# luisdiaz1997/GPzoo

Measured on AMD Instinct MI355X. Metric: ELBO evals/sec (L=32-latent evaluations, all GPUs) at M=2048 inducing, N=200000, L=32 latents/GPU x 1 GPU(s), higher is better.
Workload: dtype f32; 1 GPU; BASELINE configs[2]: Slide-seq-shaped synthetic, N=200000 spots, M=2048, L=32 latents/GPU x 1 GPU(s), matern32, f32; latents_total=32, whitened=True, chunk=0, factor_dtype=f64

## Files before the change

### gpzoo_amd/csrc/gemmw.hip

```cpp
#include "gemmw.h"

#include "cov.h"


#include <cmath>
#include <mutex>
#include <type_traits>
#include <utility>

#ifndef GPZ_W_ABL
#define GPZ_W_ABL 0
#endif

namespace gpz {

typedef float f32x4 __attribute__((ext_vector_type(4)));

enum { WB_MEM = 0, WB_GEN = 1 };
enum { WA_DENSE = 0, WA_LOWER = 1, WA_UPPER = 2 };
enum { WE_STORE_STATS = 0,
       WE_STATS = 1,
       WE_STORE = 2,
       WE_STORE_COLSCALE = 3,
       WE_WBAR = 4,
       WE_KBAR = 5,
       WE_ADD_COLSCALE = 6 };

struct WParams {
  const float* A; int64_t lda, sA0;
  const float* B; int64_t ldb, sB0;
  const float* Z; int64_t MD;
  const float* X; int64_t nreal;
  const float* sigma; const float* ell;
  float* C; int64_t ldc, sC0;
  const float* mu; int64_t sMu;
  float* ps_sq; float* ps_mu; int64_t ncols;
  const float* colscale; const float* colvec; int64_t sCs;
  const float* rowvec; int64_t sRv;
  const float* aux;
  int64_t M;
  int L, nblk, mtw, nt, W, strips;
  int pair, colmajor;
  const int32_t* gate;
};

constexpr int W_BK = 16;

template <int TM, int TN, int BSRC, int D>
struct WLds {
  static constexpr int A_ELEMS = TM * W_BK;
  static constexpr int RPP = 256 / TN;
  static constexpr int PITCH = 256 + (RPP == 2 ? 8 : RPP == 1 ? 4 : 16);
  static constexpr int B_ELEMS = (W_BK / RPP) * PITCH;
  static constexpr int STAGE = A_ELEMS + B_ELEMS;
  static constexpr int ZB = 128 * D;
  static constexpr size_t bytes = sizeof(float) * (2 * STAGE + (BSRC == WB_GEN ? 2 * ZB : 0));
};

template <int TM, int TN, int BSRC, int ATRI, int EPI, int KIND, int D>
__global__ __launch_bounds__(64 * (TM / 128) * (TN / 32)) __attribute__((amdgpu_waves_per_eu(4, 4))) void gemmw_kernel(const WParams p) {
  constexpr int BK = W_BK;
  if (p.gate && *p.gate == 0) return;
  constexpr int WMW = TM / 128, WNW = TN / 32;
  constexpr int NW = WMW * WNW;
  static_assert(NW == 8 || NW == 16, "8 or 16 waves of 128 x 32");
  using G = WLds<TM, TN, BSRC, D>;
  constexpr int RPP = G::RPP, PITCH = G::PITCH;
  extern __shared__ __attribute__((aligned(1024))) char smem_raw[];
  float* const smem = reinterpret_cast<float*>(smem_raw);
  auto sA = [&](int buf) -> float* { return smem + buf * G::STAGE; };
  auto sB = [&](int buf) -> float* { return smem + buf * G::STAGE + G::A_ELEMS; };
  float* const sZ = smem + 2 * G::STAGE;
  auto addrB = [](int k, int n) { return (k / RPP) * PITCH + (k % RPP) * TN + n; };

  int tj, b0, leg_ti[2], nlegs = 1;
  {
    const int bid = blockIdx.x;
    const int x = bid & 7, s = bid >> 3;
    if (BSRC == WB_GEN) {
      const int ug = s / p.W, within = s - ug * p.W;
      const int u = ug * 8 + x;
      const int per_level = p.L * p.strips;
      if (u >= p.mtw * per_level) return;
      const int level = u / per_level, rem = u - level * per_level;
      leg_ti[0] = leg_ti[1] = (ATRI == WA_LOWER) ? p.mtw - 1 - level : level;
      b0 = rem / p.strips;
      tj = (rem - b0 * p.strips) * p.W + within;
    } else {
      const int per_unit = (p.pair ? (p.mtw + 1) >> 1 : p.mtw) * p.W;
      const int u = (s / per_unit) * 8 + x, within = s % per_unit;
      if (u >= p.L * p.strips) return;
      b0 = u / p.strips;
      const int nrow = p.pair ? (p.mtw + 1) >> 1 : p.mtw;
      const int pi = p.colmajor ? within % nrow : within / p.W, far = p.pair ? p.mtw - 1 - pi : pi;
      const int strip = u - b0 * p.strips, c0 = strip * p.nt / p.strips, c1 = (strip + 1) * p.nt / p.strips;
      tj = c0 + (p.colmajor ? within / nrow : within % p.W);
      if (tj >= c1) return;
      const bool long_first = ((s >> 5) & 1) == 0;
      leg_ti[0] = ((ATRI == WA_LOWER) == long_first) ? far : pi;
      leg_ti[1] = ((ATRI == WA_LOWER) == long_first) ? pi : far;
      nlegs = far == pi ? 1 : 2;
      if (!p.pair) leg_ti[0] = leg_ti[1] = (ATRI == WA_LOWER) ? p.mtw - 1 - pi : pi;
    }
    if (tj >= p.nt) return;
  }
  const int tid = threadIdx.x, lane = tid & 63;
  const int wave = __builtin_amdgcn_readfirstlane(tid >> 6);
  const int wn = wave % WNW;
  const int r = lane & 15, q = lane >> 4;
  const int Mp = p.nblk * 128;

  typedef __attribute__((address_space(3))) void lds_void;
  constexpr int NPA = TM / (16 * NW);
#if defined(__HIP_DEVICE_COMPILE__)
  const __amdgpu_buffer_rsrc_t a_rsrc = __builtin_amdgcn_make_buffer_rsrc(
      const_cast<float*>(p.A + b0 * p.sA0), 0, (int)(p.lda * Mp * sizeof(float)), 0x00020000);
  const __amdgpu_buffer_rsrc_t b_rsrc = __builtin_amdgcn_make_buffer_rsrc(
      const_cast<float*>(BSRC == WB_MEM ? p.B + b0 * p.sB0 : p.Z), 0,
      (int)((BSRC == WB_MEM ? p.ldb * Mp : p.MD) * sizeof(float)), 0x00020000);
#endif
  auto k_begin_of = [&](int ti) { return (ATRI == WA_UPPER) ? TM * ti : 0; };
  auto k_end_of = [&](int ti) { return (ATRI == WA_LOWER) ? min(TM * (ti + 1), Mp) : Mp; };
  int a_soff[NPA], b_soff = 0;
  auto gperm = [](int w) { const int t = (w >> 2) & 3; return (((t >> 1) ^ t) & 1) << 1 | (t >> 1); };
  const int a_voff = ((lane >> 2) * (int)p.lda + (((lane & 3) ^ gperm(lane >> 2)) * 4)) * (int)sizeof(float);
  const int b_voff = ((lane / (TN / 4)) * (int)p.ldb + (lane % (TN / 4)) * 4) * (int)sizeof(float);
  bool abl_first = true;
  auto stage_load = [&](int buf) __attribute__((always_inline)) {
    if ((GPZ_W_ABL & 2) && !abl_first) return;
    abl_first = false;
#if defined(__HIP_DEVICE_COMPILE__)
#pragma unroll
    for (int h = 0; h < NPA; ++h) {
      __builtin_amdgcn_raw_ptr_buffer_load_lds(a_rsrc, (lds_void*)(sA(buf) + (NPA * wave + h) * 256), 16, a_voff, a_soff[h], 0, 0);
      a_soff[h] += BK * (int)sizeof(float);
    }
    if constexpr (BSRC == WB_MEM) {
      constexpr int NPB = (W_BK / RPP) / NW;
      static_assert(BSRC != WB_MEM || (NPB * NW * RPP == W_BK && NPB >= 1), "whole B pieces per wave");
#pragma unroll
      for (int h = 0; h < NPB; ++h)
        __builtin_amdgcn_raw_ptr_buffer_load_lds(b_rsrc, (lds_void*)(sB(buf) + (wave + NW * h) * PITCH), 16, b_voff,
                                                 b_soff + h * NW * RPP * (int)p.ldb * (int)sizeof(float), 0, 0);
      b_soff += BK * (int)p.ldb * (int)sizeof(float);
    }
#endif
  };
  auto tile_begin = [&](int ti) __attribute__((always_inline)) {
    const int kb = k_begin_of(ti);
#pragma unroll
    for (int h = 0; h < NPA; ++h) {
      int row = ti * TM + (NPA * wave + h) * 16;
      while (row >= Mp) row -= 128;
      a_soff[h] = (row * (int)p.lda + kb) * (int)sizeof(float);
    }
    b_soff = ((kb + RPP * wave) * (int)p.ldb + tj * TN) * (int)sizeof(float);
    stage_load(0);
  };

  constexpr int NXC = TN / 64;
  float xc[NXC][D], ampn[NXC], c0n[NXC];
  CovConst cc = {0.f, 0.f, 0.f};
  if constexpr (BSRC == WB_GEN) {
    cc = cov_const<KIND>(p.sigma[b0], p.ell[b0]);
#pragma unroll
    for (int h = 0; h < NXC; ++h) {
      const int64_t n = (int64_t)tj * TN + h * 64 + lane;
      const bool real = n < p.nreal;
#pragma unroll
      for (int k = 0; k < D; ++k) xc[h][k] = real ? p.X[n * D + k] : 0.f;
      ampn[h] = real ? cc.amp : 0.f;
      c0n[h] = (KIND == 1 && !real) ? 0.f : cc.c0;
    }
  }
  auto z_load = [&](int blk) __attribute__((always_inline)) {
#if defined(__HIP_DEVICE_COMPILE__)
    if (wave < 2 * D)
      __builtin_amdgcn_raw_ptr_buffer_load_lds(b_rsrc, (lds_void*)(sZ + (blk & 1) * G::ZB + wave * 64), 4, lane * 4,
                                               (blk * G::ZB + wave * 64) * 4, 0, 0);
#endif
  };
  auto b_generate = [&](int buf, int step) __attribute__((always_inline)) {
#pragma unroll
    for (int i = 0; i < BK / NW; ++i) {
      const int kk = wave + NW * i, kg = step * BK + kk;
      const float* zp = sZ + ((kg >> 7) & 1) * G::ZB + (kg & 127) * D;
      float z[D];
#pragma unroll
      for (int k = 0; k < D; ++k) z[k] = zp[k];
#pragma unroll
      for (int h = 0; h < NXC; ++h) {
        const float v = (GPZ_W_ABL & 1) ? z[0] + xc[h][0]
                                        : cov_value<KIND>(cov_radial<KIND>(cov_d2<D>(z, xc[h])), ampn[h], c0n[h], cc.c1);
        sB(buf)[addrB(kk, h * 64 + lane)] = v;
      }
    }
  };

  f32x4 acc[8][2];

  int wm = 0, nk = 0, db = 0, n_a = 0, fr_a = 0, step0 = 0, t = 0, next_ti = -1;
  bool active = false;
  int fr_b[4];
#pragma unroll
  for (int j = 0; j < 4; ++j) fr_b[j] = addrB(4 * q + j, wn * 32 + r);

  auto mma_step = [&](int buf, auto lo_c, auto hi_c) __attribute__((always_inline)) {
    constexpr int LO = decltype(lo_c)::value, HI = decltype(hi_c)::value;
    float bf[4][2];
#pragma unroll
    for (int j = 0; j < 4; ++j)
#pragma unroll
      for (int ni = 0; ni < 2; ++ni) bf[j][ni] = sB(buf)[fr_b[j] + ni * 16];
#pragma unroll
    for (int half = 0; half < 2; ++half) {
      f32x4 fa[4];
#pragma unroll
      for (int m = 0; m < 4; ++m)
        if (half * 4 + m >= LO && half * 4 + m <= HI)
          fa[m] = *reinterpret_cast<const f32x4*>(sA(buf) + fr_a + (half * 4 + m) * 16 * BK);
#pragma unroll
      for (int j = 0; j < 4; ++j)
#pragma unroll
        for (int m = 0; m < 4; ++m)
#pragma unroll
          for (int ni = 0; ni < 2; ++ni)
            if (half * 4 + m >= LO && half * 4 + m <= HI)
              acc[half * 4 + m][ni] = __builtin_amdgcn_mfma_f32_16x16x4f32(fa[m][j], bf[j][ni], acc[half * 4 + m][ni], 0, 0, 0);
    }
  };

  using std::integral_constant;
  auto step = [&](auto par_c, auto run_c, auto lo_c, auto hi_c) __attribute__((always_inline)) {
    constexpr int P = decltype(par_c)::value;
    if (t + 1 < nk) {
      stage_load(P ^ 1);
      if constexpr (BSRC == WB_GEN) {
        const int st = step0 + t;
        if ((st & 7) == 0 && (st >> 3) + 1 < p.nblk) z_load((st >> 3) + 1);
        b_generate(P ^ 1, st + 1);
      }
    } else if (next_ti >= 0) {
      tile_begin(next_ti);
    }
    if constexpr (decltype(run_c)::value) mma_step(P, lo_c, hi_c);
    if (GPZ_W_ABL & 16) {
      asm volatile("s_waitcnt lgkmcnt(0)" ::: "memory");
      __builtin_amdgcn_s_barrier();
    } else {
      asm volatile("s_waitcnt vmcnt(0)" ::: "memory");
      if (!(GPZ_W_ABL & 8)) __syncthreads();
    }
    ++t;
  };
  using no_run = integral_constant<bool, false>;
  using run = integral_constant<bool, true>;
  using i0 = integral_constant<int, 0>;
  using i1 = integral_constant<int, 1>;
  using i7 = integral_constant<int, 7>;
  auto idle_until = [&](int end) __attribute__((always_inline)) {
    while (t < end) { step(i0{}, no_run{}, i0{}, i7{}); step(i1{}, no_run{}, i0{}, i7{}); }
  };
  auto full_until = [&](int end) __attribute__((always_inline)) {
    while (t < end) { step(i0{}, run{}, i0{}, i7{}); step(i1{}, run{}, i0{}, i7{}); }
  };
  auto diagonal = [&](auto self, auto u_c) __attribute__((always_inline)) -> void {
    constexpr int U = decltype(u_c)::value;
    if constexpr (ATRI == WA_LOWER) step(integral_constant<int, U & 1>{}, run{}, integral_constant<int, U>{}, i7{});
    else step(integral_constant<int, U & 1>{}, run{}, i0{}, integral_constant<int, U>{});
    if constexpr (U + 1 < 8) self(self, integral_constant<int, U + 1>{});
  };

  tile_begin(leg_ti[0]);
#pragma unroll 1
  for (int leg = 0; leg < nlegs; ++leg) {
    const int ti = leg_ti[leg];
    wm = WMW == 1 ? 0 : (wave / WNW) ^ ((ti ^ tj) & 1);
    const int k_begin = k_begin_of(ti);
    nk = (k_end_of(ti) - k_begin) / BK;
    db = WMW * ti + wm;
    active = db < p.nblk && (int64_t)tj * TN + wn * 32 < p.ncols;
    n_a = 8 * (ATRI == WA_LOWER ? db : wm);
    fr_a = (wm * 128 + r) * BK + ((q ^ gperm(r)) * 4);
    step0 = k_begin / BK;
    t = 0;
    next_ti = leg + 1 < nlegs ? leg_ti[leg + 1] : -1;
#pragma unroll
    for (int mi = 0; mi < 8; ++mi)
#pragma unroll
      for (int ni = 0; ni < 2; ++ni) acc[mi][ni] = f32x4{0, 0, 0, 0};
    if constexpr (BSRC == WB_GEN) {
      z_load(step0 >> 3);
      asm volatile("s_waitcnt vmcnt(0)" ::: "memory");
      __syncthreads();
      b_generate(0, step0);
    }
    if (leg == 0) asm volatile("s_waitcnt vmcnt(0)" ::: "memory");
    asm volatile("s_waitcnt lgkmcnt(0)" ::: "memory");
    __builtin_amdgcn_s_barrier();
    if (!active) {
      idle_until(nk);
    } else if constexpr (ATRI == WA_DENSE) {
      full_until(nk);
    } else if constexpr (ATRI == WA_LOWER) {
      full_until(n_a);
      diagonal(diagonal, i0{});
      idle_until(nk);
    } else {
      idle_until(n_a);
      diagonal(diagonal, i0{});
      full_until(nk);
    }

    if (!active) continue;
    if (GPZ_W_ABL & 4) {
      float sum = 0.f;
#pragma unroll
      for (int mi = 0; mi < 8; ++mi)
#pragma unroll
        for (int ni = 0; ni < 2; ++ni)
#pragma unroll
          for (int g = 0; g < 4; ++g) sum += acc[mi][ni][g];
      if (sum == 12345.678f) p.ps_sq[0] = sum;
      continue;
    }
    const int64_t row0 = (int64_t)db * 128;
    const int64_t ccol0 = (int64_t)tj * TN + wn * 32;
    if (BSRC == WB_GEN && row0 + 128 > p.M) {
#pragma unroll
      for (int mi = 0; mi < 8; ++mi)
#pragma unroll
        for (int g = 0; g < 4; ++g)
          if (row0 + mi * 16 + 4 * q + g >= p.M) {
#pragma unroll
            for (int ni = 0; ni < 2; ++ni) acc[mi][ni][g] = 0.f;
          }
    }
    if constexpr (EPI == WE_STORE_STATS || EPI == WE_STATS) {
      float ssq[2] = {0.f, 0.f}, smu[2] = {0.f, 0.f};
#pragma unroll
      for (int mi = 0; mi < 8; ++mi) {
        f32x4 m4 = {0, 0, 0, 0};
        if constexpr (EPI == WE_STORE_STATS) m4 = *reinterpret_cast<const f32x4*>(p.mu + b0 * p.sMu + row0 + 4 * q + mi * 16);
#pragma unroll
        for (int g = 0; g < 4; ++g)
#pragma unroll
          for (int ni = 0; ni < 2; ++ni) {
            const float v = acc[mi][ni][g];
            ssq[ni] = __builtin_fmaf(v, v, ssq[ni]);
            if constexpr (EPI == WE_STORE_STATS) smu[ni] = __builtin_fmaf(m4[g], v, smu[ni]);
          }
      }
#pragma unroll
      for (int ni = 0; ni < 2; ++ni) {
        ssq[ni] += __shfl_xor(ssq[ni], 16); ssq[ni] += __shfl_xor(ssq[ni], 32);
        if constexpr (EPI == WE_STORE_STATS) { smu[ni] += __shfl_xor(smu[ni], 16); smu[ni] += __shfl_xor(smu[ni], 32); }
        if (q == 0) {
          const int64_t o = ((int64_t)b0 * p.nblk + db) * p.ncols + ccol0 + ni * 16 + r;
          p.ps_sq[o] = ssq[ni];
          if constexpr (EPI == WE_STORE_STATS) p.ps_mu[o] = smu[ni];
        }
      }
    }
    if constexpr (EPI != WE_STATS) {
      constexpr int LDE = 36;
      static_assert(NW * 16 * LDE <= G::STAGE, "the epilogue strips fit tile buffer 1");
      float* strip = sA(1) + wave * (16 * LDE);
      float* Cg = p.C + b0 * p.sC0 + row0 * p.ldc + ccol0;
      int srow = lane >> 3;
      asm volatile("" : "+v"(srow));
      const int c4 = (lane & 7) * 4;
      float cs[2] = {1.f, 1.f};
      if constexpr (EPI == WE_STORE_COLSCALE) {
#pragma unroll
        for (int ni = 0; ni < 2; ++ni) cs[ni] = p.colscale[b0 * p.sCs + ccol0 + ni * 16 + r];
      }
      f32x4 sc = {0, 0, 0, 0}, cv = {0, 0, 0, 0};
      if constexpr (EPI == WE_WBAR || EPI == WE_KBAR || EPI == WE_ADD_COLSCALE)
        sc = *reinterpret_cast<const f32x4*>(p.colscale + b0 * p.sCs + ccol0 + c4);
      if constexpr (EPI == WE_WBAR || EPI == WE_KBAR)
        cv = *reinterpret_cast<const f32x4*>(p.colvec + b0 * p.sCs + ccol0 + c4);
#pragma unroll
      for (int mi = 0; mi < 8; ++mi) {
#pragma unroll
        for (int ni = 0; ni < 2; ++ni)
#pragma unroll
          for (int g = 0; g < 4; ++g) strip[(4 * q + g) * LDE + ni * 16 + r] = cs[ni] * acc[mi][ni][g];
        __builtin_amdgcn_wave_barrier();
        f32x4 w[2];
        float rv[2];
        if constexpr (EPI == WE_WBAR || EPI == WE_KBAR || EPI == WE_ADD_COLSCALE) {
#pragma unroll
          for (int it = 0; it < 2; ++it) {
            const int64_t row = mi * 16 + it * 8 + srow;
            if constexpr (EPI == WE_WBAR) w[it] = *reinterpret_cast<const f32x4*>(p.aux + b0 * p.sC0 + (row0 + row) * p.ldc + ccol0 + c4);
            if constexpr (EPI == WE_ADD_COLSCALE) w[it] = *reinterpret_cast<const f32x4*>(Cg + (int64_t)row * p.ldc + c4);
            if constexpr (EPI != WE_ADD_COLSCALE) rv[it] = p.rowvec[b0 * p.sRv + row0 + row];
          }
        }
#pragma unroll
        for (int it = 0; it < 2; ++it) {
          const int row = it * 8 + srow;
          f32x4 v = *reinterpret_cast<const f32x4*>(strip + row * LDE + c4);
          if constexpr (EPI == WE_WBAR) {
#pragma unroll
            for (int e = 0; e < 4; ++e) v[e] = v[e] + rv[it] * cv[e] - w[it][e] * sc[e];
          }
          if constexpr (EPI == WE_KBAR) {
#pragma unroll
            for (int e = 0; e < 4; ++e) v[e] = v[e] * sc[e] + rv[it] * cv[e];
          }
          if constexpr (EPI == WE_ADD_COLSCALE) {
#pragma unroll
            for (int e = 0; e < 4; ++e) v[e] = w[it][e] + v[e] * sc[e];
          }
          *reinterpret_cast<f32x4*>(Cg + (int64_t)(mi * 16 + row) * p.ldc + c4) = v;
        }
        __builtin_amdgcn_wave_barrier();
      }
    }
  }
}

struct NTParams {
  const float* A; const float* B; float* C;
  int64_t ld, sAB, ldc, sC;
  int K, nblk, mt, L, T;
  int S, Ks;
  float* part; int64_t sPart;
  const float* w; int64_t sW;
  const int32_t* gate;
  const float* gm; float* vpart;
};

template <int TM, bool WTS>
__global__ __launch_bounds__(TM * 2) __attribute__((amdgpu_waves_per_eu(4, 4))) void gemmw_nt_kernel(const NTParams p) {
  constexpr int BK = W_BK, TN = 128;
  if (p.gate && *p.gate == 0) return;
  constexpr int NW = TM / 32;
  constexpr int A_ELEMS = TM * BK, B_ELEMS = TN * BK, STAGE = A_ELEMS + B_ELEMS;
  extern __shared__ __attribute__((aligned(1024))) char smem_raw[];
  float* const smem = reinterpret_cast<float*>(smem_raw);
  auto sA = [&](int buf) -> float* { return smem + buf * STAGE; };
  auto sB = [&](int buf) -> float* { return smem + buf * STAGE + A_ELEMS; };
  int b0, ti, tj, piece;
  {
    const int nb = (int)gridDim.x, qn = nb >> 3, rem = nb & 7, x = blockIdx.x & 7;
    const int lid0 = x * qn + min(x, rem) + (int)(blockIdx.x >> 3);
    const int grp = lid0 / p.T;
    const int t = lid0 - grp * p.T;
    b0 = grp / p.S;
    piece = grp - b0 * p.S;
    if constexpr (TM == 256) {
      int i = (int)((sqrtf(4.0f * (float)t + 1.0f) - 1.0f) * 0.5f);
      while ((i + 1) * (i + 2) <= t) ++i;
      while (i * (i + 1) > t) --i;
      ti = i; tj = t - i * (i + 1);
    } else {
      int i = (int)((sqrtf(8.0f * (float)t + 1.0f) - 1.0f) * 0.5f);
      while ((i + 1) * (i + 2) / 2 <= t) ++i;
      while (i * (i + 1) / 2 > t) --i;
      ti = i; tj = t - i * (i + 1) / 2;
    }
  }
  const int tid = threadIdx.x, lane = tid & 63;
  const int wave = __builtin_amdgcn_readfirstlane(tid >> 6);
  const int wm = wave >> 2, wn = wave & 3;
  const int r = lane & 15, q = lane >> 4;
  const int Mp = p.nblk * 128;
  const int db = (TM / 128) * ti + wm;
  const bool active = db < p.nblk && tj <= db;
  const bool same = TM == 128 && p.A == p.B && tj == ti;
  typedef __attribute__((address_space(3))) void lds_void;
#if defined(__HIP_DEVICE_COMPILE__)
  const __amdgpu_buffer_rsrc_t a_rsrc = __builtin_amdgcn_make_buffer_rsrc(
      const_cast<float*>(p.A + b0 * p.sAB), 0, (int)(p.ld * Mp * sizeof(float)), 0x00020000);
  const __amdgpu_buffer_rsrc_t b_rsrc = __builtin_amdgcn_make_buffer_rsrc(
      const_cast<float*>(p.B + b0 * p.sAB), 0, (int)(p.ld * Mp * sizeof(float)), 0x00020000);
#endif
  auto gperm = [](int w) { const int t = (w >> 2) & 3; return (((t >> 1) ^ t) & 1) << 1 | (t >> 1); };
  const int voff = ((lane >> 2) * (int)p.ld + (((lane & 3) ^ gperm(lane >> 2)) * 4)) * (int)sizeof(float);
  int a_soff[2], b_soff;
#pragma unroll
  for (int h = 0; h < 2; ++h) {
    int row = ti * TM + (2 * wave + h) * 16;
    while (row >= Mp) row -= 128;
    a_soff[h] = (row * (int)p.ld + piece * p.Ks) * (int)sizeof(float);
  }
  constexpr int NPB = 8 / NW;
  b_soff = ((tj * TN + wave * NPB * 16) * (int)p.ld + piece * p.Ks) * (int)sizeof(float);
  auto stage_load = [&](int buf) __attribute__((always_inline)) {
#if defined(__HIP_DEVICE_COMPILE__)
#pragma unroll
    for (int h = 0; h < 2; ++h) {
      __builtin_amdgcn_raw_ptr_buffer_load_lds(a_rsrc, (lds_void*)(sA(buf) + (2 * wave + h) * 256), 16, voff, a_soff[h], 0, 0);
      a_soff[h] += BK * (int)sizeof(float);
    }
    if (!same) {
#pragma unroll
      for (int h = 0; h < NPB; ++h)
        __builtin_amdgcn_raw_ptr_buffer_load_lds(b_rsrc, (lds_void*)(sB(buf) + (wave * NPB + h) * 256), 16, voff,
                                                 b_soff + h * 16 * (int)p.ld * (int)sizeof(float), 0, 0);
      b_soff += BK * (int)sizeof(float);
    }
#endif
  };
  const float* wk = WTS ? p.w + b0 * p.sW + (int64_t)piece * p.Ks + 4 * (lane >> 4) : nullptr;
  f32x4 wv;
  auto w_load = [&]() __attribute__((always_inline)) {
    if constexpr (WTS) { wv = *reinterpret_cast<const f32x4*>(wk); wk += BK; }
  };
  const int fr_a = (wm * 128 + r) * BK + ((q ^ gperm(r)) * 4);
  const int nk = (min(p.K, (piece + 1) * p.Ks) - piece * p.Ks) / BK;
  const bool split = p.S > 1;
  const bool diag = WTS && p.A == p.B && db == tj && db < p.nblk;
  if (diag) {
    auto diag_path = [&](auto wn_c) __attribute__((always_inline)) {
      constexpr int C0 = decltype(wn_c)::value, C1 = 7 - C0, N0 = 8 - C0, N1 = 8 - C1;
      const bool rd = p.gm != nullptr;
      const float* gk = rd ? p.gm + b0 * p.sW + (int64_t)piece * p.Ks + 4 * (lane >> 4) : nullptr;
      f32x4 gv = f32x4{0, 0, 0, 0};
      float pv0 = 0.f, pv1 = 0.f;
      f32x4 a0[N0], a1[N1];
#pragma unroll
      for (int i = 0; i < N0; ++i) a0[i] = f32x4{0, 0, 0, 0};
#pragma unroll
      for (int i = 0; i < N1; ++i) a1[i] = f32x4{0, 0, 0, 0};
      const int fb_off = r * BK + ((q ^ gperm(r)) * 4) + (same ? -A_ELEMS : 0);
      auto step = [&](int buf, bool more) __attribute__((always_inline)) {
        f32x4 f0 = *reinterpret_cast<const f32x4*>(sB(buf) + fb_off + C0 * 16 * BK);
        f32x4 f1 = *reinterpret_cast<const f32x4*>(sB(buf) + fb_off + C1 * 16 * BK);
        f0 *= wv; f1 *= wv;
        if (more) w_load();
#pragma unroll
        for (int mi = C0; mi < 8; ++mi) {
          const f32x4 fa = *reinterpret_cast<const f32x4*>(sA(buf) + fr_a + mi * 16 * BK);
#pragma unroll
          for (int j = 0; j < 4; ++j) {
            a0[mi - C0] = __builtin_amdgcn_mfma_f32_16x16x4f32(fa[j], f0[j], a0[mi - C0], 0, 0, 0);
            if (mi >= C1) a1[mi >= C1 ? mi - C1 : 0] = __builtin_amdgcn_mfma_f32_16x16x4f32(fa[j], f1[j], a1[mi >= C1 ? mi - C1 : 0], 0, 0, 0);
          }
          if (mi == 2 * C0 || mi == 2 * C0 + 1) {
            if (rd) {
              const f32x4 t = fa * gv;
              if (mi == 2 * C0) pv0 += (t[0] + t[1]) + (t[2] + t[3]); else pv1 += (t[0] + t[1]) + (t[2] + t[3]);
            }
          }
        }
        if (more && rd) { gv = *reinterpret_cast<const f32x4*>(gk); gk += BK; }
      };
      if (rd) { gv = *reinterpret_cast<const f32x4*>(gk); gk += BK; }
      stage_load(0);
      w_load();
      asm volatile("s_waitcnt vmcnt(0)" ::: "memory");
      __syncthreads();
      for (int t = 0; t < nk; t += 2) {
        if (t + 1 < nk) stage_load(1);
        step(0, t + 1 < nk);
        asm volatile("s_waitcnt vmcnt(0)" ::: "memory");
        __syncthreads();
        if (t + 2 < nk) stage_load(0);
        step(1, t + 2 < nk);
        asm volatile("s_waitcnt vmcnt(0)" ::: "memory");
        __syncthreads();
      }
      if (rd) {
        float* vp = p.vpart + ((int64_t)piece * p.L + b0) * Mp + db * 128;
        pv0 += __shfl_xor(pv0, 16); pv0 += __shfl_xor(pv0, 32);
        pv1 += __shfl_xor(pv1, 16); pv1 += __shfl_xor(pv1, 32);
        if (q == 0) { vp[(2 * C0) * 16 + r] = pv0; vp[(2 * C0 + 1) * 16 + r] = pv1; }
      }
      float* Cg = (split ? p.part + piece * p.sPart : p.C) + b0 * p.sC + (int64_t)db * 128 * p.ldc + (int64_t)tj * TN;
      auto put = [&](const f32x4& a, int mi, int c) __attribute__((always_inline)) {
        float* o = Cg + (int64_t)(mi * 16 + 4 * q) * p.ldc + c * 16 + r;
#pragma unroll
        for (int g = 0; g < 4; ++g) o[g * p.ldc] = split ? a[g] : o[g * p.ldc] + a[g];
      };
#pragma unroll
      for (int mi = C0; mi < 8; ++mi) put(a0[mi - C0], mi, C0);
#pragma unroll
      for (int mi = C1; mi < 8; ++mi) put(a1[mi - C1], mi, C1);
    };
    switch (wn) {
      case 0: diag_path(std::integral_constant<int, 0>{}); break;
      case 1: diag_path(std::integral_constant<int, 1>{}); break;
      case 2: diag_path(std::integral_constant<int, 2>{}); break;
      default: diag_path(std::integral_constant<int, 3>{}); break;
    }
    return;
  }
  f32x4 acc[8][2];
#pragma unroll
  for (int mi = 0; mi < 8; ++mi)
#pragma unroll
    for (int ni = 0; ni < 2; ++ni) acc[mi][ni] = f32x4{0, 0, 0, 0};
  const int fr_b = (wn * 32 + r) * BK + ((q ^ gperm(r)) * 4) + (same ? -A_ELEMS : 0);
  auto mma_step = [&](int buf, bool more) __attribute__((always_inline)) {
    f32x4 fb[2];
#pragma unroll
    for (int ni = 0; ni < 2; ++ni) {
      fb[ni] = *reinterpret_cast<const f32x4*>(sB(buf) + fr_b + ni * 16 * BK);
      if constexpr (WTS) fb[ni] *= wv;
    }
    if (more) w_load();
#pragma unroll
    for (int half = 0; half < 2; ++half) {
      f32x4 fa[4];
#pragma unroll
      for (int m = 0; m < 4; ++m) fa[m] = *reinterpret_cast<const f32x4*>(sA(buf) + fr_a + (half * 4 + m) * 16 * BK);
#pragma unroll
      for (int j = 0; j < 4; ++j)
#pragma unroll
        for (int m = 0; m < 4; ++m)
#pragma unroll
          for (int ni = 0; ni < 2; ++ni)
            acc[half * 4 + m][ni] = __builtin_amdgcn_mfma_f32_16x16x4f32(fa[m][j], fb[ni][j], acc[half * 4 + m][ni], 0, 0, 0);
    }
  };
  stage_load(0);
  w_load();
  asm volatile("s_waitcnt vmcnt(0)" ::: "memory");
  __syncthreads();
  if (active) {
    for (int t = 0; t < nk; t += 2) {
      if (t + 1 < nk) stage_load(1);
      mma_step(0, t + 1 < nk);
      asm volatile("s_waitcnt vmcnt(0)" ::: "memory");
      __syncthreads();
      if (t + 2 < nk) stage_load(0);
      mma_step(1, t + 2 < nk);
      asm volatile("s_waitcnt vmcnt(0)" ::: "memory");
      __syncthreads();
    }
  } else {
    for (int t = 0; t < nk; t += 2) {
      if (t + 1 < nk) stage_load(1);
      asm volatile("s_waitcnt vmcnt(0)" ::: "memory");
      __syncthreads();
      if (t + 2 < nk) stage_load(0);
      asm volatile("s_waitcnt vmcnt(0)" ::: "memory");
      __syncthreads();
    }
    return;
  }
  constexpr int LDE = 36;
  float* strip = smem + wave * (32 * LDE);
  float* Cg = (split ? p.part + piece * p.sPart : p.C) + b0 * p.sC + (int64_t)db * 128 * p.ldc + (int64_t)tj * TN + wn * 32;
  const int srow = lane >> 3, c4 = (lane & 7) * 4;
#pragma unroll
  for (int pass = 0; pass < 4; ++pass) {
#pragma unroll
    for (int mm = 0; mm < 2; ++mm)
#pragma unroll
      for (int ni = 0; ni < 2; ++ni)
#pragma unroll
        for (int g = 0; g < 4; ++g) strip[(mm * 16 + 4 * q + g) * LDE + ni * 16 + r] = acc[pass * 2 + mm][ni][g];
    __builtin_amdgcn_wave_barrier();
    f32x4 cin[4];
#pragma unroll
    for (int it = 0; it < 4; ++it)
      cin[it] = split ? f32x4{0, 0, 0, 0} : *reinterpret_cast<const f32x4*>(Cg + (int64_t)(pass * 32 + it * 8 + srow) * p.ldc + c4);
#pragma unroll
    for (int it = 0; it < 4; ++it) {
      const int row = it * 8 + srow;
      const f32x4 v = *reinterpret_cast<const f32x4*>(strip + row * LDE + c4);
      *reinterpret_cast<f32x4*>(Cg + (int64_t)(pass * 32 + row) * p.ldc + c4) = cin[it] + v;
    }
    __builtin_amdgcn_wave_barrier();
  }
}

__global__ __launch_bounds__(256) void nt_reduce_kernel(float* __restrict__ C, const float* __restrict__ part, int S, int64_t sPart,
                                                        int Mp, int64_t total4, const int32_t* __restrict__ gate, int sym) {
  const int64_t i4 = (int64_t)blockIdx.x * 256 + threadIdx.x;
  if (i4 >= total4 || (gate && *gate == 0)) return;
  const int64_t e = i4 * 4;
  const int col = (int)(e % Mp), row = (int)((e / Mp) % Mp);
  if ((col >> 7) > (row >> 7) || (sym && (col >> 4) > (row >> 4))) return;
  f32x4 v = *reinterpret_cast<const f32x4*>(C + e);
  for (int s = 0; s < S; ++s) v += *reinterpret_cast<const f32x4*>(part + s * sPart + e);
  *reinterpret_cast<f32x4*>(C + e) = v;
}

__global__ __launch_bounds__(256) void nt_vsum_kernel(const float* __restrict__ vpart, int S, int64_t LM, double* __restrict__ v,
                                                      int64_t Mp, int64_t v_stride) {
  const int64_t i = (int64_t)blockIdx.x * 256 + threadIdx.x;
  if (i >= LM) return;
  double t = 0.0;
  for (int s = 0; s < S; ++s) t += (double)vpart[s * LM + i];
  v[(i / Mp) * v_stride + i % Mp] = t;
}

template <typename K>
static int launch_wide(K kernel, size_t lds, const WParams& p, int64_t nblocks, hipStream_t s, int threads = 512) {
  struct Seen { const void* fn; int dev; };
  static Seen seen[64];
  static int n_seen = 0;
  static std::mutex mu;
  int dev = 0;
  GPZ_HIP_OK(hipGetDevice(&dev));
  if (lds > 64 * 1024) {
    const void* fn = reinterpret_cast<const void*>(kernel);
    std::lock_guard<std::mutex> lock(mu);
    bool have = false;
    for (int i = 0; i < n_seen; ++i) have = have || (seen[i].fn == fn && seen[i].dev == dev);
    if (!have) {
      GPZ_HIP_OK(hipFuncSetAttribute(fn, hipFuncAttributeMaxDynamicSharedMemorySize, (int)lds));
      if (n_seen < 64) seen[n_seen++] = Seen{fn, dev};
    }
  }
  GPZ_REQUIRE(nblocks > 0 && nblocks < (1ll << 31), "wide product: bad grid");
  hipLaunchKernelGGL(kernel, dim3((unsigned)nblocks), dim3((unsigned)threads), lds, s, p);
  GPZ_LAUNCH_OK();
  return 0;
}

bool fused1_supported(int dtype, int kind, int d) {
  return dtype == GPZ_F32 && (kind == GPZ_KERNEL_RBF || kind == GPZ_KERNEL_MATERN32) && (d == 1 || d == 2);
}

int fused1_launch(const Fused1Args& a, hipStream_t s) {
  GPZ_REQUIRE(fused1_supported(GPZ_F32, a.kind, a.d), "fused stage 1: kind=%d d=%d unsupported", a.kind, a.d);
  GPZ_REQUIRE(a.Mp % 128 == 0 && a.ncp % 128 == 0 && a.Mp > 0 && a.ncp > 0 && a.L > 0, "fused stage 1: bad extents");
  GPZ_REQUIRE(a.Mp * a.Mp * 4 < (1ll << 31) && a.M * a.d * 4 < (1ll << 31), "fused stage 1: M too large");
  constexpr int TM = 512, TN = 128;
  WParams p = {};
  p.A = a.Linv; p.lda = a.Mp; p.sA0 = a.Mp * a.Mp;
  p.Z = a.Z; p.MD = a.M * a.d; p.M = a.M;
  p.X = a.X; p.nreal = a.nreal;
  p.sigma = a.sigma; p.ell = a.ell;
  p.C = a.Wt; p.ldc = a.ncp; p.sC0 = a.Mp * a.ncp;
  p.mu = a.muE; p.sMu = a.Mp;
  p.ps_sq = a.ps_sq; p.ps_mu = a.ps_mu; p.ncols = a.ncp;
  p.L = a.L; p.nblk = (int)(a.Mp / 128); p.mtw = (int)((a.Mp + TM - 1) / TM); p.nt = (int)(a.ncp / TN);
  int strips = (p.nt + 31) / 32;
  const int want = (32 + p.mtw * p.L - 1) / (p.mtw * p.L);
  if (strips < want) strips = want < p.nt ? want : p.nt;
  p.W = (p.nt + strips - 1) / strips;
  p.strips = (p.nt + p.W - 1) / p.W;
  const int64_t units = (int64_t)p.mtw * p.L * p.strips;
  const int64_t nblocks = (units + 7) / 8 * 8 * p.W;
#define GPZ_W1(KIND, D) return launch_wide(gemmw_kernel<TM, TN, WB_GEN, WA_LOWER, WE_STORE_STATS, KIND, D>, \
                                           WLds<TM, TN, WB_GEN, D>::bytes, p, nblocks, s, 1024)
  if (a.kind == GPZ_KERNEL_MATERN32) { if (a.d == 2) GPZ_W1(1, 2); GPZ_W1(1, 1); }
  if (a.d == 2) GPZ_W1(0, 2);
  GPZ_W1(0, 1);
#undef GPZ_W1
}

bool wide_product_supported(int64_t Mp, int64_t ncp) {
  return Mp % 128 == 0 && ncp % 128 == 0 && Mp * Mp * 4 < (1ll << 31) && Mp * ncp * 4 < (1ll << 31);
}

template <int TM, int TN>
static int wide_product_launch_t(const WideArgs& a, hipStream_t s) {
  WParams p = {};
  p.A = a.A; p.lda = a.Mp; p.sA0 = a.Mp * a.Mp;
  p.B = a.B; p.ldb = a.ncp; p.sB0 = a.Mp * a.ncp;
  p.C = a.C; p.ldc = a.ncp; p.sC0 = a.Mp * a.ncp;
  p.mu = a.mu; p.sMu = a.Mp;
  p.ps_sq = a.ps_sq; p.ps_mu = a.ps_mu; p.ncols = a.ncp; p.M = a.Mp;
  p.colscale = a.colscale; p.colvec = a.colvec; p.sCs = a.ncp; p.rowvec = a.rowvec; p.sRv = a.Mp; p.aux = a.aux;
  p.gate = a.gate;
  p.L = a.L; p.nblk = (int)(a.Mp / 128); p.mtw = (int)((a.Mp + TM - 1) / TM); p.nt = (int)((a.ncp + TN - 1) / TN);
  constexpr int WMAX = 4096 / TN;
  int strips = (p.nt + WMAX - 1) / WMAX;
  const int want = (8 + p.L - 1) / p.L;
  if (strips < want) strips = want < p.nt ? want : p.nt;
  p.strips = strips;
  p.W = (p.nt + strips - 1) / strips;
  const int64_t units = (int64_t)p.L * p.strips;
  const int64_t paired = (units + 7) / 8 * 8 * ((p.mtw + 1) / 2) * p.W;
  p.pair = p.colmajor = paired >= 4 * 512;
  const int64_t nblocks = p.pair ? paired : (units + 7) / 8 * 8 * p.mtw * p.W;
  constexpr size_t lds = WLds<TM, TN, WB_MEM, 1>::bytes;
#define GPZ_WM(ATRI, EPI) return launch_wide(gemmw_kernel<TM, TN, WB_MEM, ATRI, EPI, 0, 1>, lds, p, nblocks, s)
  switch (a.epilogue) {
    case WIDE_STORE_STATS:
      GPZ_REQUIRE(!a.upper && a.C && a.mu && a.ps_sq && a.ps_mu, "wide product: store + statistics is the lower-triangular product and needs C, mu and both slabs");
      GPZ_WM(WA_LOWER, WE_STORE_STATS);
    case WIDE_STATS:
      GPZ_REQUIRE(a.upper && a.ps_sq, "wide product: statistics only is the upper-triangular product");
      GPZ_WM(WA_UPPER, WE_STATS);
    case WIDE_STORE:
      GPZ_REQUIRE(a.upper && a.C, "wide product: the plain store is built for the upper-triangular product");
      GPZ_WM(WA_UPPER, WE_STORE);
    case WIDE_STORE_COLSCALE:
      GPZ_REQUIRE(a.upper && a.C && a.colscale, "wide product: the column-scaled store is the upper-triangular product and needs the factors");
      GPZ_WM(WA_UPPER, WE_STORE_COLSCALE);
    case WIDE_WBAR:
      GPZ_REQUIRE(!a.upper && a.C && a.colscale && a.colvec && a.rowvec && a.aux, "wide product: the W-bar epilogue needs its operands");
      GPZ_WM(WA_LOWER, WE_WBAR);
    case WIDE_KBAR:
      GPZ_REQUIRE(a.upper == 2 && a.C && a.colscale && a.colvec && a.rowvec, "wide product: the K-bar epilogue is the dense product and needs its vectors");
      GPZ_WM(WA_DENSE, WE_KBAR);
    case WIDE_ADD_COLSCALE:
      GPZ_REQUIRE(a.upper == 1 && a.C && a.colscale, "wide product: the accumulating column-scaled store is the upper-triangular product");
      GPZ_WM(WA_UPPER, WE_ADD_COLSCALE);
    default: break;
  }
#undef GPZ_WM
  GPZ_REQUIRE(false, "wide product: unknown epilogue %d", a.epilogue);
}

int wide_product_launch(const WideArgs& a, hipStream_t s) {
  GPZ_REQUIRE(wide_product_supported(a.Mp, a.ncp) && a.L > 0, "wide product: bad extents");
  return wide_product_launch_t<128, 256>(a, s);
}

bool wide_nt_supported(int64_t Mp, int64_t K) {
  return Mp % 128 == 0 && K % 128 == 0 && K > 0 && Mp * K * 4 < (1ll << 31);
}

static bool nt_small_tiles(int64_t nblk) { return nblk <= 4; }
static int64_t nt_tiles(int64_t nblk) {
  if (nt_small_tiles(nblk)) return nblk * (nblk + 1) / 2;
  const int64_t mt = (nblk + 1) / 2;
  return mt * (mt + 1) - (nblk & 1);
}

int wide_nt_pieces(int64_t Mp, int64_t K, int L) {
  const int64_t tiles = nt_tiles(Mp / 128) * L;
  if (tiles >= 384) {
    const double r = (double)tiles / 512.0;
    int best = 1;
    double best_cost = 1e30;
    for (int S = 1; S <= 4; ++S) {
      if (S > 1 && K / S < 2048) break;
      const double rounds = r * S, cost = std::ceil(rounds - 1e-9) / rounds * (1.0 + 0.015 * (S - 1));
      if (cost < best_cost - 1e-9) { best_cost = cost; best = S; }
    }
    return best;
  }
  int64_t S = (nt_small_tiles(Mp / 128) ? 1024 : 512) / tiles;
  S = std::min<int64_t>(S, K / 1024);
  S = std::min<int64_t>(S, 16);
  return (int)std::max<int64_t>(S, 1);
}

size_t wide_nt_vpart_floats(int64_t Mp, int64_t K, int L) { return (size_t)wide_nt_pieces(Mp, K, L) * L * Mp; }

size_t wide_nt_scratch_floats(int64_t Mp, int64_t K, int L) {
  const int S = wide_nt_pieces(Mp, K, L);
  return S > 1 ? (size_t)S * L * Mp * Mp : 0;
}

int wide_nt_launch(const float* A, const float* B, float* C, int64_t Mp, int64_t K, int L, hipStream_t s, float* scratch,
                   const float* w, const int32_t* gate, const float* gm, float* vpart, double* v, int64_t v_stride) {
  GPZ_REQUIRE(A && B && C && wide_nt_supported(Mp, K) && L > 0, "wide A B^T: bad arguments");
  GPZ_REQUIRE(!gm || (w && vpart && v && A == B), "wide A B^T: the row products A gm need weights, A == B and their buffers");
  NTParams p;
  p.w = w; p.sW = K; p.gate = gate; p.gm = gm; p.vpart = vpart;
  p.A = A; p.B = B; p.C = C; p.ld = K; p.sAB = Mp * K; p.ldc = Mp; p.sC = Mp * Mp;
  p.K = (int)K; p.nblk = (int)(Mp / 128); p.mt = (p.nblk + 1) / 2; p.L = L;
  const bool small = nt_small_tiles(p.nblk);
  p.T = (int)nt_tiles(p.nblk);
  int S = scratch ? wide_nt_pieces(Mp, K, L) : 1;
  p.Ks = (int)(((K + S - 1) / S + 31) / 32 * 32);
  S = (int)((K + p.Ks - 1) / p.Ks);
  p.S = S; p.part = scratch; p.sPart = (int64_t)L * Mp * Mp;
  const int64_t nblocks = (int64_t)p.T * L * S;
  GPZ_REQUIRE(nblocks > 0 && nblocks < (1ll << 31), "wide A B^T: bad grid");
  if (small) {
    constexpr size_t lds = sizeof(float) * 2 * (128 + 128) * W_BK;
    if (w) hipLaunchKernelGGL((gemmw_nt_kernel<128, true>), dim3((unsigned)nblocks), dim3(256), lds, s, p);
    else hipLaunchKernelGGL((gemmw_nt_kernel<128, false>), dim3((unsigned)nblocks), dim3(256), lds, s, p);
  } else {
    constexpr size_t lds = sizeof(float) * 2 * (256 + 128) * W_BK;
    if (w) hipLaunchKernelGGL((gemmw_nt_kernel<256, true>), dim3((unsigned)nblocks), dim3(512), lds, s, p);
    else hipLaunchKernelGGL((gemmw_nt_kernel<256, false>), dim3((unsigned)nblocks), dim3(512), lds, s, p);
  }
  GPZ_LAUNCH_OK();
  if (S > 1) {
    const int64_t total4 = (int64_t)L * Mp * Mp / 4;
    hipLaunchKernelGGL(nt_reduce_kernel, dim3((unsigned)((total4 + 255) / 256)), dim3(256), 0, s, C, scratch, S, p.sPart, (int)Mp, total4, gate, (int)(w != nullptr && A == B));
    GPZ_LAUNCH_OK();
  }
  if (gm) {
    const int64_t LM = (int64_t)L * Mp;
    hipLaunchKernelGGL(nt_vsum_kernel, dim3((unsigned)((LM + 255) / 256)), dim3(256), 0, s, vpart, S, LM, v, Mp, v_stride);
    GPZ_LAUNCH_OK();
  }
  return 0;
}

}
```

Measured before the change: 2.641 ELBO evals/s.

## Add 256x256 diagonal superblock tiles for symmetric weighted A·Aᵀ products

For the symmetric weighted NT product with large tile counts, the tile schedule now gives diagonal blocks as single 256x256 superblocks that load only A into LDS and compute the lower triangle across 8 waves. This cuts the number of diagonal tiles and skips the redundant B loads. Off-diagonal tiles are re-indexed to match. The split-K piece count is recomputed for the new tile count. Scratch sizing takes the max of the two schedules. Risks are per-wave load imbalance inside superblocks, since waves own different column strips of the triangle, and higher register pressure from the per-wave accumulators.

```diff
diff --git a/gpzoo_amd/csrc/gemmw.hip b/gpzoo_amd/csrc/gemmw.hip
--- a/gpzoo_amd/csrc/gemmw.hip
+++ b/gpzoo_amd/csrc/gemmw.hip
@@ -4,6 +4,8 @@
 
 
 #include <cmath>
+#include <cstdlib>
+#include <cstring>
 #include <mutex>
 #include <type_traits>
 #include <utility>
@@ -431,6 +433,7 @@
   const float* w; int64_t sW;
   const int32_t* gate;
   const float* gm; float* vpart;
+  int sb;
 };
 
 template <int TM, bool WTS>
@@ -444,6 +447,7 @@
   auto sA = [&](int buf) -> float* { return smem + buf * STAGE; };
   auto sB = [&](int buf) -> float* { return smem + buf * STAGE + A_ELEMS; };
   int b0, ti, tj, piece;
+  bool sbd = false;
   {
     const int nb = (int)gridDim.x, qn = nb >> 3, rem = nb & 7, x = blockIdx.x & 7;
     const int lid0 = x * qn + min(x, rem) + (int)(blockIdx.x >> 3);
@@ -452,10 +456,23 @@
     b0 = grp / p.S;
     piece = grp - b0 * p.S;
     if constexpr (TM == 256) {
+      if (WTS && p.sb) {
+        const int nd = p.nblk >> 1;
+        if (t < nd) { ti = t; tj = 2 * t; sbd = true; }
+        else {
+          const int u = t - nd;
+          int i = (int)((sqrtf(4.0f * (float)u + 1.0f) + 1.0f) * 0.5f);
+          while (i * (i + 1) <= u) ++i;
+          while (i * (i - 1) > u) --i;
+          i = min(i, p.mt - 1);
+          ti = i; tj = u - i * (i - 1);
+        }
+      } else {
       int i = (int)((sqrtf(4.0f * (float)t + 1.0f) - 1.0f) * 0.5f);
       while ((i + 1) * (i + 2) <= t) ++i;
       while (i * (i + 1) > t) --i;
       ti = i; tj = t - i * (i + 1);
+      }
     } else {
       int i = (int)((sqrtf(8.0f * (float)t + 1.0f) - 1.0f) * 0.5f);
       while ((i + 1) * (i + 2) / 2 <= t) ++i;
@@ -496,7 +513,7 @@
       __builtin_amdgcn_raw_ptr_buffer_load_lds(a_rsrc, (lds_void*)(sA(buf) + (2 * wave + h) * 256), 16, voff, a_soff[h], 0, 0);
       a_soff[h] += BK * (int)sizeof(float);
     }
-    if (!same) {
+    if (!same && !sbd) {
 #pragma unroll
       for (int h = 0; h < NPB; ++h)
         __builtin_amdgcn_raw_ptr_buffer_load_lds(b_rsrc, (lds_void*)(sB(buf) + (wave * NPB + h) * 256), 16, voff,
@@ -505,14 +522,96 @@
     }
 #endif
   };
-  const float* wk = WTS ? p.w + b0 * p.sW + (int64_t)piece * p.Ks + 4 * (lane >> 4) : nullptr;
+  const int kq = 4 * (lane >> 4);
+  const float* wk = WTS ? p.w + b0 * p.sW + (int64_t)piece * p.Ks : nullptr;
   f32x4 wv;
   auto w_load = [&]() __attribute__((always_inline)) {
-    if constexpr (WTS) { wv = *reinterpret_cast<const f32x4*>(wk); wk += BK; }
+    if constexpr (WTS) { wv = *reinterpret_cast<const f32x4*>(wk + kq); wk += BK; }
   };
   const int fr_a = (wm * 128 + r) * BK + ((q ^ gperm(r)) * 4);
   const int nk = (min(p.K, (piece + 1) * p.Ks) - piece * p.Ks) / BK;
   const bool split = p.S > 1;
+  if constexpr (TM == 256 && WTS) {
+    if (sbd) {
+      auto sb_path = [&](auto w_c) __attribute__((always_inline)) {
+        constexpr int C0 = decltype(w_c)::value, C1 = 15 - C0, N0 = 16 - C0, N1 = 16 - C1;
+        const bool rd = p.gm != nullptr;
+        const float* gk = rd ? p.gm + b0 * p.sW + (int64_t)piece * p.Ks : nullptr;
+        f32x4 gv = f32x4{0, 0, 0, 0};
+        float pv0 = 0.f, pv1 = 0.f;
+        f32x4 a0[N0], a1[N1];
+#pragma unroll
+        for (int i = 0; i < N0; ++i) a0[i] = f32x4{0, 0, 0, 0};
+#pragma unroll
+        for (int i = 0; i < N1; ++i) a1[i] = f32x4{0, 0, 0, 0};
+        const int fr = r * BK + ((q ^ gperm(r)) * 4);
+        auto step = [&](int buf, bool more) __attribute__((always_inline)) {
+          f32x4 f0 = *reinterpret_cast<const f32x4*>(sA(buf) + fr + C0 * 16 * BK);
+          f32x4 f1 = *reinterpret_cast<const f32x4*>(sA(buf) + fr + C1 * 16 * BK);
+          f0 *= wv; f1 *= wv;
+          if (more) w_load();
+#pragma unroll
+          for (int mi = C0; mi < 16; ++mi) {
+            const f32x4 fa = *reinterpret_cast<const f32x4*>(sA(buf) + fr + mi * 16 * BK);
+#pragma unroll
+            for (int j = 0; j < 4; ++j) {
+              a0[mi - C0] = __builtin_amdgcn_mfma_f32_16x16x4f32(fa[j], f0[j], a0[mi - C0], 0, 0, 0);
+              if (mi >= C1) a1[mi >= C1 ? mi - C1 : 0] = __builtin_amdgcn_mfma_f32_16x16x4f32(fa[j], f1[j], a1[mi >= C1 ? mi - C1 : 0], 0, 0, 0);
+            }
+            if (mi == 2 * C0 || mi == 2 * C0 + 1) {
+              if (rd) {
+                const f32x4 t = fa * gv;
+                if (mi == 2 * C0) pv0 += (t[0] + t[1]) + (t[2] + t[3]); else pv1 += (t[0] + t[1]) + (t[2] + t[3]);
+              }
+            }
+          }
+          if (more && rd) { gv = *reinterpret_cast<const f32x4*>(gk + kq); gk += BK; }
+        };
+        if (rd) { gv = *reinterpret_cast<const f32x4*>(gk + kq); gk += BK; }
+        stage_load(0);
+        w_load();
+        asm volatile("s_waitcnt vmcnt(0)" ::: "memory");
+        __syncthreads();
+        for (int t = 0; t < nk; t += 2) {
+          if (t + 1 < nk) stage_load(1);
+          step(0, t + 1 < nk);
+          asm volatile("s_waitcnt vmcnt(0)" ::: "memory");
+          __syncthreads();
+          if (t + 2 < nk) stage_load(0);
+          step(1, t + 2 < nk);
+          asm volatile("s_waitcnt vmcnt(0)" ::: "memory");
+          __syncthreads();
+        }
+        if (rd) {
+          float* vp = p.vpart + ((int64_t)piece * p.L + b0) * Mp + ti * 256;
+          pv0 += __shfl_xor(pv0, 16); pv0 += __shfl_xor(pv0, 32);
+          pv1 += __shfl_xor(pv1, 16); pv1 += __shfl_xor(pv1, 32);
+          if (q == 0) { vp[(2 * C0) * 16 + r] = pv0; vp[(2 * C0 + 1) * 16 + r] = pv1; }
+        }
+        float* Cg = (split ? p.part + piece * p.sPart : p.C) + b0 * p.sC + (int64_t)ti * 256 * p.ldc + (int64_t)ti * 256;
+        auto put = [&](const f32x4& a, int mi, int c) __attribute__((always_inline)) {
+          float* o = Cg + (int64_t)(mi * 16 + 4 * q) * p.ldc + c * 16 + r;
+#pragma unroll
+          for (int g = 0; g < 4; ++g) o[g * p.ldc] = split ? a[g] : o[g * p.ldc] + a[g];
+        };
+#pragma unroll
+        for (int mi = C0; mi < 16; ++mi) put(a0[mi - C0], mi, C0);
+#pragma unroll
+        for (int mi = C1; mi < 16; ++mi) put(a1[mi - C1], mi, C1);
+      };
+      switch (wave) {
+        case 0: sb_path(std::integral_constant<int, 0>{}); break;
+        case 1: sb_path(std::integral_constant<int, 1>{}); break;
+        case 2: sb_path(std::integral_constant<int, 2>{}); break;
+        case 3: sb_path(std::integral_constant<int, 3>{}); break;
+        case 4: sb_path(std::integral_constant<int, 4>{}); break;
+        case 5: sb_path(std::integral_constant<int, 5>{}); break;
+        case 6: sb_path(std::integral_constant<int, 6>{}); break;
+        default: sb_path(std::integral_constant<int, 7>{}); break;
+      }
+      return;
+    }
+  }
   const bool diag = WTS && p.A == p.B && db == tj && db < p.nblk;
   if (diag) {
     auto diag_path = [&](auto wn_c) __attribute__((always_inline)) {
@@ -813,14 +912,19 @@
 }
 
 static bool nt_small_tiles(int64_t nblk) { return nblk <= 4; }
-static int64_t nt_tiles(int64_t nblk) {
+static bool nt_superblocks(int64_t nblk, bool sym) {
+  static const bool env_split = [] { const char* e = getenv("GPZ_NT_DIAG"); return e && !strcmp(e, "split"); }();
+  return sym && !nt_small_tiles(nblk) && !env_split;
+}
+static int64_t nt_tiles(int64_t nblk, bool sym) {
   if (nt_small_tiles(nblk)) return nblk * (nblk + 1) / 2;
   const int64_t mt = (nblk + 1) / 2;
+  if (nt_superblocks(nblk, sym)) return nblk / 2 + mt * (mt - 1) + (nblk & 1);
   return mt * (mt + 1) - (nblk & 1);
 }
 
-int wide_nt_pieces(int64_t Mp, int64_t K, int L) {
-  const int64_t tiles = nt_tiles(Mp / 128) * L;
+static int nt_pieces(int64_t Mp, int64_t K, int L, bool sym) {
+  const int64_t tiles = nt_tiles(Mp / 128, sym) * L;
   if (tiles >= 384) {
     const double r = (double)tiles / 512.0;
     int best = 1;
@@ -838,6 +942,8 @@
   return (int)std::max<int64_t>(S, 1);
 }
 
+int wide_nt_pieces(int64_t Mp, int64_t K, int L) { return std::max(nt_pieces(Mp, K, L, false), nt_pieces(Mp, K, L, true)); }
+
 size_t wide_nt_vpart_floats(int64_t Mp, int64_t K, int L) { return (size_t)wide_nt_pieces(Mp, K, L) * L * Mp; }
 
 size_t wide_nt_scratch_floats(int64_t Mp, int64_t K, int L) {
@@ -853,9 +959,10 @@
   p.w = w; p.sW = K; p.gate = gate; p.gm = gm; p.vpart = vpart;
   p.A = A; p.B = B; p.C = C; p.ld = K; p.sAB = Mp * K; p.ldc = Mp; p.sC = Mp * Mp;
   p.K = (int)K; p.nblk = (int)(Mp / 128); p.mt = (p.nblk + 1) / 2; p.L = L;
-  const bool small = nt_small_tiles(p.nblk);
-  p.T = (int)nt_tiles(p.nblk);
-  int S = scratch ? wide_nt_pieces(Mp, K, L) : 1;
+  const bool small = nt_small_tiles(p.nblk), sym = w != nullptr && A == B;
+  p.sb = nt_superblocks(p.nblk, sym);
+  p.T = (int)nt_tiles(p.nblk, sym);
+  int S = scratch ? nt_pieces(Mp, K, L, sym) : 1;
   p.Ks = (int)(((K + S - 1) / S + 31) / 32 * 32);
   S = (int)((K + p.Ks - 1) / p.Ks);
   p.S = S; p.part = scratch; p.sPart = (int64_t)L * Mp * Mp;
```

Result: no change. 2.643 ELBO evals/s, median of 3 (+0.1%).
